# slowkow/harmonypy

Hardware: AMD Instinct MI355X
Metric: cells/sec/Harmony-iteration (higher is better)
Workload: dtype f32; 1 GPU; BASELINE configs[2] (C3): 1000000 cells x 50 PCs, 8 batches, K=100 per GPU; step = 1 Harmony iteration = 10 k-means rounds (block_size 0.05 -> 20 blocks) + 1 ridge correction; cells_per_gpu=1000000, pcs=50, batches=8, clusters=100, update_order=device (keyed bijection, generated inside the timed region), init=k-means++ on a 50k-cell subsample, untimed, parallelism=single GPU, cells_total=1000000

## Files before the change

### harmonypy_amd/_capi.py

```python
from __future__ import annotations

import ctypes as C
import os

import numpy as np

_HERE = os.path.dirname(os.path.abspath(__file__))
LIB_PATH = os.environ.get("HMX_LIB") or os.path.join(_HERE, "libhmx.so")

HMX_TILE = 16
HMX_MAX_CLUSTERS, HMX_MAX_PCS, HMX_MAX_BLOCKS, HMX_MAX_VARS = 320, 320, 250, 32
HMX_Z_ORIG, HMX_Z_COS, HMX_Z_CORR, HMX_R, HMX_Y, HMX_O_GROUP, HMX_T_MASS, HMX_W = range(8)
HMX_ROUND_BLOCK_START, HMX_ROUND_CELLS, HMX_ROUND_TILE_GROUP = 8, 9, 10
HMX_ROUND_CENTROIDS, HMX_ROUND_UPDATE_R, HMX_ROUND_OBJECTIVE = 1, 2, 4
HMX_ROUND_ALL = 7
HMX_DTYPE_F32, HMX_DTYPE_F16, HMX_DTYPE_BF16, HMX_DTYPE_F64 = range(4)

EXPORTS = [
    "hmx_last_error", "hmx_abi_version", "hmx_create", "hmx_destroy", "hmx_upload", "hmx_init_cluster",
    "hmx_cluster_round", "hmx_cluster_round_seeded", "hmx_moe_correct_ridge", "hmx_get", "hmx_set", "hmx_sync", "hmx_device_ptr",
    "hmx_kernel_times", "hmx_enable_timing", "hmx_counters", "hmx_comm_unique_id", "hmx_comm_init", "hmx_set_host_allreduce",
    "hmx_build_id", "hmx_cluster", "hmx_set_timing_stride", "hmx_set_timing_families", "hmx_kmeans_lloyd", "hmx_can_lloyd", "hmx_kmeans_seed", "hmx_compute_lisi", "hmx_get_rows", "hmx_set_ranks", "hmx_peer_export", "hmx_peer_attach", "hmx_peer_selftest", "hmx_peer_enable",
]
DEVICE_IO_EXPORTS = ["hmx_upload_device", "hmx_copy_out_device", "hmx_compute_lisi_device"]
# ... 310 lines not shown
        shape, dt = self._shape(which)
        out = np.empty(shape, dt)
        _check(self._lib.hmx_get(self._h, which, _ptr(out), out.nbytes))
        return out

    def get_rows(self, which, rows):
        rows = _c(rows, np.int32)
        shape, dt = self._shape(which)
        assert dt == np.float32
        out = np.empty((len(rows), shape[1]), np.float32)
        _check(self._lib.hmx_get_rows(self._h, which, _ptr(rows), len(rows), _ptr(out), out.nbytes))
        return out

    def set(self, which, arr):
        shape, dt = self._shape(which)
        arr = _c(arr, dt)
        assert arr.shape == tuple(shape), (arr.shape, shape)
        _check(self._lib.hmx_set(self._h, which, _ptr(arr), arr.nbytes))

    def round_lists(self):
        bs = np.empty(self.nblk + 1, np.int32)
        _check(self._lib.hmx_get(self._h, HMX_ROUND_BLOCK_START, _ptr(bs), bs.nbytes))
        nt = int(bs[-1])
        cells = np.empty(nt * HMX_TILE, np.int32)
        tg = np.empty(nt, np.int32)
        if nt:
            _check(self._lib.hmx_get(self._h, HMX_ROUND_CELLS, _ptr(cells), cells.nbytes))
            _check(self._lib.hmx_get(self._h, HMX_ROUND_TILE_GROUP, _ptr(tg), tg.nbytes))
        return cells, tg, bs

    def sync(self):
        _check(self._lib.hmx_sync(self._h))

    @staticmethod
    def comm_unique_id() -> bytes:
        buf = C.create_string_buffer(HMX_UNIQUE_ID_BYTES)
        _check(load().hmx_comm_unique_id(buf))
        return buf.raw

    def enable_timing(self, on=True, families=None, stride=1):
        _check(self._lib.hmx_set_timing_stride(self._h, int(stride)))
        if on:
            mask = 0xFFFFFFFF if families is None else sum(1 << KERNEL_FAMILIES.index(f) for f in families)
            _check(self._lib.hmx_set_timing_families(self._h, mask))
        _check(self._lib.hmx_enable_timing(self._h, 1 if on else 0))

    def counters(self):
        buf = np.zeros(16, np.int64)
        _check(self._lib.hmx_counters(self._h, _ptr(buf)))
        return {"collectives": int(buf[0]), "sweep_fallbacks": int(buf[1]), "seeded_rounds": int(buf[2]), "sweeps_bf16_pipe": int(buf[3]),
                "sweep_waits": int(buf[4]), "sweep_wait_polls": int(buf[5]), "sweep_wait_polls_max": int(buf[6]), "rtz_bf16_pipe": int(buf[7]),
                "sweeps_group_affine": int(buf[8]), "sweep_group_affine_wgs": int(buf[9]),
                "peer_box": {0: "none", 1: "coarse", 2: "fine"}[int(buf[10])], "rtz_presplit_z": int(buf[11]),
                "sweeps_wide_persistent": int(buf[12]), "rtz_task_tiles_max": int(buf[13])}

    def kernel_times(self):
        buf = np.zeros(2 * len(KERNEL_FAMILIES), np.float64)
        _check(self._lib.hmx_kernel_times(self._h, _ptr(buf), buf.size, None))
        return {n: (float(buf[2 * i]), int(buf[2 * i + 1])) for i, n in enumerate(KERNEL_FAMILIES)}
```

### harmonypy_amd/csrc/hmx_capi.cpp

```cpp
#include <hip/hip_runtime.h>
#include <dlfcn.h>

#include <algorithm>
#include <climits>
#include <cmath>
#include <cstdarg>
#include <cstdio>
#include <cstdlib>
#include <cstring>
#include <functional>
#include <string>
#include <vector>

#include "hmx.h"
#include "hmx_device_io.h"
#include "hmx_knn.h"
#include "hmx_map.h"
#include "hmx_score.h"
#include "hmx_internal.h"
#include "hmx_score_kernels.h"
#ifdef RTZ_PROF
void rtz_prof_dump();
#endif

// ... 55 lines not shown
    hipStream_t s;
    ~SyncOnExit() { (void)hipStreamSynchronize(s); }
};

}

struct hmx_engine {
    hmx_config cfg{};
    int64_t N = 0;
    int d = 0, dp = 0, K = 0, Kp = 0, K16 = 0, mt = 0, ntd = 0, ldy = 0, B = 0, G = 0, V = 0, nblk = 0;
    int max_wgs = 1024;
    hipStream_t stream = nullptr;
    bool uploaded = false, clustered = false, timing = false;
    unsigned timing_mask = ~0u;
    int timing_stride = 1;
    long fam_seen[8] = {0};

    DevBuf<float> Zorig, Zcos, Zcorr, R, Y, Yacc, sigma, theta, Pr_b, lamb, rp, lrp, slab, W;
    DevBuf<int> group_cols, s_cells, s_tile_grp, task_t0, task_t1, task_grp;
    struct Lists { DevBuf<int> cells, tile_grp, blk_start, run_tiles; bool runs_ok = false; };
    Lists lists[2];
    int cur = 0;
    hipStream_t stream2 = nullptr;
    hipEvent_t pre_event = nullptr;
    bool pre_valid = false;
    bool pre_outstanding = false;
    uint64_t pre_seed = 0, pre_counter = 0;
    int64_t pre_cpb = 0;
    DevBuf<int> gstart, chunk_tab, run_count, run_start, global_id;
    DevBuf<int> cell_map, cell_inv;
    bool map_perm = true, inv_valid = false;
    hipEvent_t io_ev[2] = {nullptr, nullptr};
    uint64_t seeded_rounds = 0;
    int64_t Ng = 0;
    DevBuf<double> Ogrp, Tmass, Ohist, scratch;
    DevBuf<double> ref_terms;
    DevBuf<float> km_hn;
    DevBuf<double> km_sums;
    DevBuf<double> Sslots;
    unsigned* sync_words = nullptr;
    unsigned* sync_host = nullptr;
    int n_cus = 0;
    int round_mode = 1;
    unsigned spin_limit = 1u << 24;
    long n_sweep_fallbacks = 0;
    bool lists_beside_rtz = true;
    bool wide_sweep = true;
    bool wide_sweep_launched = false;
    long n_sweeps_wide = 0;
    long n_rtz_bf16 = 0;
    bool allow_round_bf16 = true;
    int rtz3_quad = 4;
    bool allow_rtz_bf16 = true;
    long n_sweeps_bf16 = 0;
    long n_sweeps_ga = 0;
    bool allow_round_ga = true;
    std::vector<int> gsize;
    DevBuf<int> ga_map;
    int ga_nwg = 0;
    int ga_per_wg = 0;
    int64_t ga_key_block = -1;
    int ga_key_cap = -1;
    bool ga_extra = false;
    DevBuf<unsigned long long> wait_stats;
    DevBuf<double> xch;
    double *Sold = nullptr, *Yacc64 = nullptr, *Snew = nullptr, *objacc = nullptr, *Sr = nullptr, *Oxr = nullptr;
    double* obj_host = nullptr;
    double* obj_defer = nullptr;
    hipEvent_t sync_event = nullptr;
    long clean_sweeps = 0;
    long n_sweep_launches = 0;
    long test_fail_sweep = -1;
    unsigned* frozen() const { return reinterpret_cast<unsigned*>(wait_stats.p + 3); }
    void* nccl_comm = nullptr;
    int n_ranks = 1, rank = 0;
    hmx_host_allreduce_fn host_fn = nullptr;
    void* host_ctx = nullptr;
    double* stage_host = nullptr;
    size_t stage_n = 0;
    long n_collectives = 0;
    double* box = nullptr;
    size_t box_doubles = 0;
    bool box_fine = false;
    std::vector<void*> peer_ptrs;
    DevBuf<double*> peer_dev;
    bool peers_attached = false, peers_enabled = false;
    unsigned long long round_epoch = 0;
    unsigned long long selftest_token = 0x5EED0000ull;
    int prefetch_lists = 1;
    int round_wgs_cap = 0;
    int n_s_tiles = 0, ntasks = 0;
    std::vector<int> h_task_grp;
    int rtz3_task_cap = 0;
    int round_req = -1;
    int rtz_kernel = 3;
    bool static_contig = false;
    int ntasks3 = 0;
    int task3_tiles_max = 0;
    DevBuf<int> t3_t0, t3_t1, t3_c0, t3_cend, t3_grp, t3_stride, s_tile_start;
    DevBuf<unsigned char> tile_blk[2], tile_blk_zero;
    DevBuf<unsigned> Yf;
    DevBuf<unsigned> Wf;
    DevBuf<unsigned> Zcf;
    bool zcf_valid = false;
    bool fuse_block_table = true;
    bool allow_zcf = true;
    long n_rtz_zf = 0;
    DevBuf<double> Opriv;
    DevBuf<double> Osave;

    struct Span { hipEvent_t a, b; int fam; };
    std::vector<Span> spans;
    std::vector<hipEvent_t> pool;
    double fam_ms[F_COUNT] = {0};
    long fam_n[F_COUNT] = {0};
};

namespace {

int use_device(hmx_engine* e) {
    HIP_TRY(hipSetDevice(e->cfg.device_id));
    return 0;
}


struct RcclApi {
    void* handle = nullptr;
    int (*GetUniqueId)(void*) = nullptr;
    int (*CommInitRank)(void**, int, hmx_nccl_id, int) = nullptr;
    int (*AllReduce)(const void*, void*, size_t, int, int, void*, hipStream_t) = nullptr;
    int (*CommDestroy)(void*) = nullptr;
    const char* (*GetErrorString)(int) = nullptr;
};
RcclApi g_rccl;

int rccl_load() {
    if (g_rccl.handle) return 0;
    const char* names[] = {getenv("HMX_RCCL_LIB"), "librccl.so.1", "/opt/rocm/lib/librccl.so.1", "librccl.so"};
    void* h = nullptr;
    std::string tried;
    for (const char* n : names) {
        if (!n || !*n) continue;
        h = dlopen(n, RTLD_NOW | RTLD_LOCAL);
        if (h) break;
        tried += std::string(" ") + n + " (" + dlerror() + ")";
    }
    if (!h) return fail(HMX_ERR_COMM, "RCCL not found:%s", tried.c_str());
    RcclApi a;
    a.handle = h;
    a.GetUniqueId = reinterpret_cast<int (*)(void*)>(dlsym(h, "ncclGetUniqueId"));
    a.CommInitRank = reinterpret_cast<int (*)(void**, int, hmx_nccl_id, int)>(dlsym(h, "ncclCommInitRank"));
    a.AllReduce = reinterpret_cast<int (*)(const void*, void*, size_t, int, int, void*, hipStream_t)>(dlsym(h, "ncclAllReduce"));
    a.CommDestroy = reinterpret_cast<int (*)(void*)>(dlsym(h, "ncclCommDestroy"));
// ... 394 lines not shown
        for (int g = 0; g < e->G; ++g) gs[g + 1] = gs[g] + gcount[g];
        if (gs[e->G] != e->N) return fail(HMX_ERR_ARG, "static list must hold every cell exactly once");
        e->gsize = gcount;
        e->ga_nwg = 0; e->ga_key_block = -1;
        if ((rc = e->gstart.reserve(e->G + 1))) return rc;
        HIP_TRY(hipMemcpyAsync(e->gstart.p, gs.data(), gs.size() * sizeof(int), hipMemcpyHostToDevice, e->stream));
        HIP_TRY(hipStreamSynchronize(e->stream));
    }
    std::vector<int> t0, t1, tg;
    const int CH = rtz2_ok(e->mt, e->dp) ? std::max(16, (n_static_tiles + 2 * HMX_RTZ2_WGS_PER_CU * e->n_cus - 1) / (2 * HMX_RTZ2_WGS_PER_CU * e->n_cus))
                   : rtz_wide_ok(e->mt, e->dp) ? std::max(16, (n_static_tiles + 2 * e->n_cus - 1) / (2 * e->n_cus)) : 64;
    for (int i = 0; i < n_static_tiles;) {
        int j = i;
        while (j < n_static_tiles && j - i < CH && static_tile_group[j] == static_tile_group[i]) ++j;
        t0.push_back(i); t1.push_back(j); tg.push_back(static_tile_group[i]);
        i = j;
    }
    for (size_t i = 1; i < tg.size(); ++i)
        if (tg[i] < tg[i - 1]) return fail(HMX_ERR_ARG, "static tiles must be sorted by group");
    e->ntasks = (int)t0.size();
    e->h_task_grp = tg;
    if ((rc = e->task_t0.reserve(t0.size())) || (rc = e->task_t1.reserve(t0.size())) || (rc = e->task_grp.reserve(t0.size()))) return rc;
    HIP_TRY(hipMemcpyAsync(e->task_t0.p, t0.data(), t0.size() * sizeof(int), hipMemcpyHostToDevice, e->stream));
    HIP_TRY(hipMemcpyAsync(e->task_t1.p, t1.data(), t1.size() * sizeof(int), hipMemcpyHostToDevice, e->stream));
    HIP_TRY(hipMemcpyAsync(e->task_grp.p, tg.data(), tg.size() * sizeof(int), hipMemcpyHostToDevice, e->stream));
    {
        bool contig = true;
        std::vector<int> tstart(e->G + 1, 0);
        for (int t = 0; t < n_static_tiles && contig; ++t) {
            const int32_t* c = static_cells + (size_t)t * HMX_TILE;
            int n = 0;
            while (n < HMX_TILE && c[n] >= 0) ++n;
            if (n == 0) { contig = false; break; }
            for (int i = 0; i < HMX_TILE; ++i)
                if (c[i] != (i < n ? c[0] + i : -1)) contig = false;
            const bool last_of_group = t + 1 == n_static_tiles || static_tile_group[t + 1] != static_tile_group[t];
            if (!last_of_group && (n < HMX_TILE || static_cells[(size_t)(t + 1) * HMX_TILE] != c[0] + HMX_TILE)) contig = false;
        }
        for (int t = 0; t < n_static_tiles; ++t) tstart[static_tile_group[t] + 1]++;
        for (int g = 0; g < e->G; ++g) tstart[g + 1] += tstart[g];
        std::vector<int> gs2(e->G + 1, 0);
        {
            std::vector<int> gcount(e->G, 0);
            for (int t = 0; t < n_static_tiles; ++t)
                for (int i = 0; i < HMX_TILE; ++i)
                    if (static_cells[(size_t)t * HMX_TILE + i] >= 0) gcount[static_tile_group[t]]++;
            for (int g = 0; g < e->G; ++g) gs2[g + 1] = gs2[g] + gcount[g];
        }
        for (int g = 0; g < e->G && contig; ++g)
            if (tstart[g + 1] > tstart[g] && static_cells[(size_t)tstart[g] * HMX_TILE] != gs2[g]) contig = false;
        e->static_contig = contig;
        e->ntasks3 = 0;
        e->task3_tiles_max = 0;
        if (contig) {
            std::vector<int> a0, a1, ac0, acend, ag, ast;
            const bool one_per_cu = e->allow_rtz_bf16 && (rtz_wide_ok(e->mt, e->dp) ? rtzw2b_ok(e->mt, e->dp, e->d, e->nblk) : rtz3b_ok(e->mt, e->dp, e->nblk, e->Kp));
            const int target = std::max(1, (one_per_cu ? 1 : 2) * e->n_cus - e->G);
            int cap3 = one_per_cu ? 4096 : 256;
            if (e->rtz3_task_cap) cap3 = e->rtz3_task_cap;
            const int CH3 = std::max(16, std::min(cap3, (n_static_tiles + target - 1) / target));
            e->rtz3_quad = rtz3_quad(e->mt, e->dp, e->nblk, e->Kp, e->allow_rtz_bf16);
            const int quad = rtz_wide_ok(e->mt, e->dp) ? 1 : e->rtz3_quad;
            for (int g = 0; g < e->G; ++g) {
                const int ts = tstart[g], te = tstart[g + 1];
                if (te <= ts) continue;
                const int m = (te - ts + CH3 - 1) / CH3;
                const int mm = std::min(m, (te - ts + quad - 1) / quad);
                const int nq = (te - ts + quad - 1) / quad, first = (nq + mm - 1) / mm;
                e->task3_tiles_max = std::max(e->task3_tiles_max, quad * first - ((nq - 1) % mm == 0 ? quad * nq - (te - ts) : 0));
                for (int j = 0; j < mm; ++j) {
                    a0.push_back(ts + quad * j); a1.push_back(te); ag.push_back(g); ast.push_back(quad * mm);
                    ac0.push_back(gs2[g] + quad * j * HMX_TILE); acend.push_back(gs2[g + 1]);
                }
            }
            e->ntasks3 = (int)a0.size();
            const size_t nt3 = a0.size();
            if ((rc = e->t3_t0.reserve(nt3)) || (rc = e->t3_t1.reserve(nt3)) || (rc = e->t3_c0.reserve(nt3)) || (rc = e->t3_cend.reserve(nt3)) || (rc = e->t3_stride.reserve(nt3)) ||
                (rc = e->t3_grp.reserve(nt3)) || (rc = e->s_tile_start.reserve(e->G + 1)) ||
                (rc = e->tile_blk[0].reserve((size_t)n_static_tiles * HMX_TILE)) || (rc = e->tile_blk[1].reserve((size_t)n_static_tiles * HMX_TILE)) ||
                (rc = e->tile_blk_zero.reserve((size_t)n_static_tiles * HMX_TILE)))
                return rc;
            HIP_TRY(hipMemcpyAsync(e->t3_t0.p, a0.data(), nt3 * sizeof(int), hipMemcpyHostToDevice, e->stream));
            HIP_TRY(hipMemcpyAsync(e->t3_t1.p, a1.data(), nt3 * sizeof(int), hipMemcpyHostToDevice, e->stream));
            HIP_TRY(hipMemcpyAsync(e->t3_c0.p, ac0.data(), nt3 * sizeof(int), hipMemcpyHostToDevice, e->stream));
            HIP_TRY(hipMemcpyAsync(e->t3_stride.p, ast.data(), nt3 * sizeof(int), hipMemcpyHostToDevice, e->stream));
            HIP_TRY(hipMemcpyAsync(e->t3_cend.p, acend.data(), nt3 * sizeof(int), hipMemcpyHostToDevice, e->stream));
            HIP_TRY(hipMemcpyAsync(e->t3_grp.p, ag.data(), nt3 * sizeof(int), hipMemcpyHostToDevice, e->stream));
            HIP_TRY(hipMemcpyAsync(e->s_tile_start.p, tstart.data(), tstart.size() * sizeof(int), hipMemcpyHostToDevice, e->stream));
            HIP_TRY(hipMemsetAsync(e->tile_blk[0].p, 255, (size_t)n_static_tiles * HMX_TILE, e->stream));
            HIP_TRY(hipMemsetAsync(e->tile_blk[1].p, 255, (size_t)n_static_tiles * HMX_TILE, e->stream));
            HIP_TRY(hipMemsetAsync(e->tile_blk_zero.p, 0, (size_t)n_static_tiles * HMX_TILE, e->stream));
            HIP_TRY(hipMemsetAsync(e->R.p + (size_t)e->N * e->Kp, 0, (size_t)16 * e->Kp * sizeof(float), e->stream));
            HIP_TRY(hipMemsetAsync(e->Zorig.p + (size_t)e->N * e->dp, 0, (size_t)16 * e->dp * sizeof(float), e->stream));
            HIP_TRY(hipMemsetAsync(e->Zcos.p + (size_t)e->N * e->dp, 0, (size_t)16 * e->dp * sizeof(float), e->stream));
            HIP_TRY(hipMemsetAsync(e->Zcorr.p + (size_t)e->N * e->dp, 0, (size_t)16 * e->dp * sizeof(float), e->stream));
            HIP_TRY(hipStreamSynchronize(e->stream));
        }
    }
    HIP_TRY(hipStreamSynchronize(e->stream));
    HIP_TRY(hipGetLastError());
    e->uploaded = true;
    return HMX_OK;
}

}

// ... 1205 lines not shown
    if (streaming_rtz(e)) {
        if ((rc = rtz3_pass(e, 1, e->tile_blk_zero.p, 1, false, false, Z))) return rc;
    } else {
    HIP_TRY(hipMemsetAsync(e->Sr, 0, GK * e->ldy * sizeof(double), e->stream));
    HIP_TRY(hipMemsetAsync(e->Oxr, 0, GK * sizeof(double), e->stream));
    {
        Timed t(e, F_RIDGE_STATS);
        RtzArgs r{};
        r.R = e->R.p; r.Z = Z; r.cells = e->s_cells.p; r.tile_grp = e->s_tile_grp.p;
        r.task_tile0 = e->task_t0.p; r.task_tile1 = e->task_t1.p; r.task_grp = e->task_grp.p;
        r.S_out = e->Oxr; r.slab = e->slab.p; r.n_tiles = e->n_s_tiles; r.ntasks = e->ntasks;
        r.K = e->K; r.Kp = e->Kp; r.K16 = e->K16; r.G = e->G; r.mt = e->mt; r.dp = e->dp; r.ntd = e->ntd;
        if (rtz2) {
            launch_rtz2(r, e->ntasks, e->stream);
            launch_rtz2_reduce(e->slab.p, e->ntasks, e->mt, e->dp, e->K16, e->ldy, e->Sr, e->task_grp.p, e->stream);
        } else if (rtzw) {
            launch_rtz_wide(r, e->ntasks, e->stream);
            launch_rtz_wide_reduce(e->slab.p, e->ntasks, e->mt, e->dp, e->K16, e->ldy, e->Sr, e->task_grp.p, e->stream);
        } else {
            launch_rtz(r, (e->ntasks + 3) / 4, e->stream);
            launch_rtz_reduce(e->slab.p, e->ntasks, e->mt, e->ntd, e->K16, e->ldy, e->Sr, e->task_grp.p, e->stream);
        }
    }
    }
    return sum_over_ranks(e, e->Sr, GK * e->ldy + GK);
}

static int ridge_solve_apply(hmx_engine* e, const double* ref_mass, const double* ref_sums) {
    int rc;
    const bool rtz2 = rtz2_ok(e->mt, e->dp);
    const bool rtzw = !rtz2 && rtz_wide_ok(e->mt, e->dp);
    {
        Timed t(e, F_RIDGE_SOLVE);
        RidgeSolveArgs s{};
        s.S = e->Sr; s.Ox = e->Oxr; s.T = e->Tmass.p; s.lamb = e->lamb.p; s.Pr_b = e->Pr_b.p; s.group_cols = e->group_cols.p;
        s.W = e->W.p; s.scratch = e->scratch.p; s.alpha = e->cfg.alpha; s.lambda_est = e->cfg.lambda_estimation;
        s.ref_mass = ref_mass; s.ref_sums = ref_sums;
        s.K = e->K; s.K16 = e->K16; s.G = e->G; s.B = e->B; s.V = e->V; s.d = e->d; s.lds = e->ldy; s.ldw = e->ldy;
        launch_ridge_solve(s, e->stream);
    }
    {
        Timed t(e, F_RIDGE_APPLY);
        ApplyArgs a{};
        a.R = e->R.p; a.Zorig = e->Zorig.p; a.W = e->W.p; a.Zcorr = e->Zcorr.p; a.Zcos = e->Zcos.p;
        a.cells = e->s_cells.p; a.tile_grp = e->s_tile_grp.p; a.n_tiles = e->n_s_tiles;
        a.Kp = e->Kp; a.K16 = e->K16; a.dp = e->dp; a.ldw = e->ldy; a.mtd = e->ntd;
        if (rtz2 || rtzw) { a.task_tile0 = e->task_t0.p; a.task_tile1 = e->task_t1.p; a.task_grp = e->task_grp.p; a.ntasks = e->ntasks; }
        e->zcf_valid = false;
        if (rtzw && e->allow_round_bf16) {
            if ((rc = e->Wf.reserve(w_planes_dwords(e->G, e->K16, e->dp)))) return rc;
            launch_w_planes(e->W.p, e->G, e->K16, e->ldy, e->dp, e->Wf.p, e->stream);
            a.Wf = e->Wf.p;
        }
        if (launch_ridge_apply(a, e->max_wgs, e->stream)) return fail(HMX_ERR_ARG, "unsupported n_pcs");
    }
    HIP_TRY(hipGetLastError());
    return HMX_OK;
}

int hmx_moe_correct_ridge(hmx_engine* e) {
    if (!e) return fail(HMX_ERR_ARG, "null argument");
    if (!e->clustered) return fail(HMX_ERR_STATE, "no soft assignment yet");
    int rc;
    if ((rc = use_device(e))) return rc;
    if ((rc = ridge_stats(e, e->Zorig.p))) return rc;
    return ridge_solve_apply(e, nullptr, nullptr);
}


int hmx_reference_summary(hmx_engine* e, double* cluster_sums_out, double* cluster_mass_out) {
    if (!e || !cluster_sums_out || !cluster_mass_out) return fail(HMX_ERR_ARG, "null argument");
    if (!e->uploaded) return fail(HMX_ERR_STATE, "hmx_upload must come first");
    if (!e->clustered) return fail(HMX_ERR_STATE, "hmx_reference_summary: no soft assignment yet");
    int rc;
    if ((rc = use_device(e))) return rc;
    if ((rc = ridge_stats(e, e->Zcorr.p))) return rc;
    const size_t GK = (size_t)e->G * e->K16, n = GK * e->ldy + GK;
    std::vector<double> h(n);
    HIP_TRY(hipStreamSynchronize(e->stream));
    HIP_TRY(hipGetLastError());
    HIP_TRY(hipMemcpy(h.data(), e->Sr, n * sizeof(double), hipMemcpyDeviceToHost));
    const double* S = h.data();
    const double* O = S + GK * e->ldy;
    for (int k = 0; k < e->K; ++k) {
        double m = 0.0;
        for (int g = 0; g < e->G; ++g) m += O[(size_t)g * e->K16 + k];
        cluster_mass_out[k] = m;
        for (int j = 0; j < e->d; ++j) {
            double v = 0.0;
            for (int g = 0; g < e->G; ++g) v += S[((size_t)g * e->K16 + k) * e->ldy + j];
            cluster_sums_out[(size_t)k * e->d + j] = v;
        }
    }
    return HMX_OK;
}

int hmx_map_query(hmx_engine* e, const double* cluster_sums, const double* cluster_mass) {
    if (!e || !cluster_sums || !cluster_mass) return fail(HMX_ERR_ARG, "null argument");
    if (!e->uploaded) return fail(HMX_ERR_STATE, "hmx_upload must come first");
    const int K = e->K, d = e->d, ldy = e->ldy, K16 = e->K16;
    std::vector<float> y0((size_t)K * d);
    std::vector<double> terms((size_t)K16 * (ldy + 1), 0.0);
    for (int k = 0; k < K; ++k) {
        const double m = cluster_mass[k];
        if (!std::isfinite(m)) return fail(HMX_ERR_ARG, "hmx_map_query: cluster_mass[%d] is not finite", k);
        terms[k] = m;
// ... 126 lines not shown
        const size_t GK = (size_t)e->G * e->K16;
        HIP_TRY(hipMemsetAsync(e->Ogrp.p, 0, GK * sizeof(double), e->stream));
        launch_group_sums(e->R.p, e->Kp, e->K, e->K16, e->s_cells.p, e->s_tile_grp.p, e->n_s_tiles, e->Ogrp.p, e->stream);
        if ((rc = sum_over_ranks(e, e->Ogrp.p, GK))) return rc;
        TableArgs ta = table_args(e);
        ta.O_prev = e->Ogrp.p; ta.T_out = e->Tmass.p;
        launch_block_table(ta, e->K16, e->stream);
        HIP_TRY(hipStreamSynchronize(e->stream));
        HIP_TRY(hipGetLastError());
        e->clustered = true;
    }
    return HMX_OK;
}

int hmx_sync(hmx_engine* e) {
    if (!e) return fail(HMX_ERR_ARG, "null argument");
    int rc;
    if ((rc = use_device(e))) return rc;
    HIP_TRY(hipStreamSynchronize(e->stream));
    HIP_TRY(hipGetLastError());
    return HMX_OK;
}

int hmx_device_ptr(hmx_engine* e, int which, void** d_ptr, size_t* bytes) {
    if (!e || !d_ptr || !bytes) return fail(HMX_ERR_ARG, "null argument");
    size_t need; int rows, cols, ld, elem, rc;
    if ((rc = locate(e, which, d_ptr, &need, &rows, &cols, &ld, &elem))) return rc;
    if (which == HMX_Z_COS) e->allow_zcf = false;
    *bytes = (size_t)rows * ld * elem;
    return HMX_OK;
}

int hmx_counters(hmx_engine* e, int64_t out[HMX_N_COUNTERS]) {
    if (!e || !out) return fail(HMX_ERR_ARG, "null argument");
    int rc;
    if ((rc = use_device(e))) return rc;
    unsigned long long ws[4] = {0, 0, 0, 0};
    HIP_TRY(hipStreamSynchronize(e->stream));
    HIP_TRY(hipMemcpy(ws, e->wait_stats.p, sizeof ws, hipMemcpyDeviceToHost));
    out[0] = e->n_collectives;
    out[1] = e->n_sweep_fallbacks;
    out[2] = (int64_t)e->seeded_rounds;
    out[3] = e->n_sweeps_bf16;
    out[4] = (int64_t)ws[0];
    out[5] = (int64_t)ws[1];
    out[6] = (int64_t)ws[2];
    out[7] = e->n_rtz_bf16;
    out[8] = e->n_sweeps_ga;
    out[9] = e->n_sweeps_ga > 0 ? e->ga_nwg : 0;
    out[10] = e->box ? (e->box_fine ? 2 : 1) : 0;
    out[11] = e->n_rtz_zf;
    out[12] = e->n_sweeps_wide;
    out[13] = e->task3_tiles_max;
    for (int i = 14; i < HMX_N_COUNTERS; ++i) out[i] = 0;
    return HMX_OK;
}

int hmx_enable_timing(hmx_engine* e, int on) {
    if (!e) return fail(HMX_ERR_ARG, "null argument");
    (void)hipSetDevice(e->cfg.device_id);
    (void)hipStreamSynchronize(e->stream);
    drain_spans(e);
    e->timing = on != 0;
    for (int i = 0; i < F_COUNT; ++i) { e->fam_ms[i] = 0; e->fam_n[i] = 0; e->fam_seen[i] = 0; }
    return HMX_OK;
}

int hmx_set_timing_families(hmx_engine* e, unsigned mask) {
    if (!e) return fail(HMX_ERR_ARG, "null argument");
    if (mask == 0) return fail(HMX_ERR_ARG, "empty family mask (hmx_enable_timing(e, 0) turns timing off)");
    e->timing_mask = mask;
    return HMX_OK;
}

int hmx_set_timing_stride(hmx_engine* e, int stride) {
    if (!e || stride < 1) return fail(HMX_ERR_ARG, "stride must be >= 1");
    e->timing_stride = stride;
    return HMX_OK;
}

int hmx_kernel_times(hmx_engine* e, double* ms_out, int n, const char** names_out) {
    if (!e || !ms_out) return fail(HMX_ERR_ARG, "null argument");
    (void)hipSetDevice(e->cfg.device_id);
    (void)hipStreamSynchronize(e->stream);
    drain_spans(e);
    for (int i = 0; i < F_COUNT && 2 * i + 1 < n; ++i) { ms_out[2 * i] = e->fam_ms[i]; ms_out[2 * i + 1] = (double)e->fam_n[i]; }
    if (names_out) *names_out = kFamilyNames;
    return F_COUNT;
}


static int score_engine_checks(hmx_engine* e, int which_Z, const char* who, const float** Z) {
    if (!e->uploaded) return fail(HMX_ERR_STATE, "%s: hmx_upload must come first", who);
    if (!e->clustered) return fail(HMX_ERR_STATE, "%s: no soft assignment yet", who);
    if (sharded(e) || e->n_ranks > 1 || e->Ng != e->N)
        return fail(HMX_ERR_STATE, "%s: this engine holds one shard of a sharded job; mapping confidence needs all cells on one engine", who);
    if (which_Z != HMX_Z_ORIG && which_Z != HMX_Z_CORR) return fail(HMX_ERR_ARG, "%s: which_Z must be HMX_Z_ORIG or HMX_Z_CORR (%d)", who, which_Z);
    *Z = which_Z == HMX_Z_ORIG ? e->Zorig.p : e->Zcorr.p;
    return 0;
}

static int score_chunks(int64_t N, size_t per_chunk, size_t budget, int cap, int64_t* chunk) {
    int64_t c = std::min<int64_t>({(N + 1023) / 1024, (int64_t)(budget / std::max<size_t>(per_chunk, 1)), (int64_t)cap});
    c = std::max<int64_t>(c, 1);
    *chunk = (((N + c - 1) / c) + 7) & ~(int64_t)7;
    return (int)((N + *chunk - 1) / *chunk);
}
// ... 135 lines not shown
```

### harmonypy_amd/csrc/hmx_internal.h

```cpp
#pragma once
#include <hip/hip_runtime.h>
#include <stddef.h>
#include <stdint.h>

#define HMX_RTZ_MTW 7
#define HMX_RTZ_NTW 4
#define HMX_OBJ_SLOTS 64

struct AssignArgs {
    const float* Zcos;
    const float* Y;
    const float* sigma;
    const float* rp;
    const float* lrp;
    float* R;
    const int* cells;
    const int* tile_grp;
    double* S_out;
    double* obj;
    const int* blk_start;
    int blk;
    int tile_begin, tile_end;
    int K, Kp, K16, mt, dp, ldy;
    int G, ldy_lds, tables_in_lds;
// ... 118 lines not shown
void launch_zplanes(const float* Z, int dp, int n_tiles, const int* tile_grp, const int* gstart, const int* s_tile_start, unsigned* Zf, hipStream_t s);
bool rtzw2b_ok(int mt, int dp, int d, int nblk);
int launch_rtzw(const Rtz3Args& a, int mt, int dp, int d, int nblk, hipStream_t s, bool allow_bf16);
void launch_tile_blocks(const int* cells, const int* tile_grp, const int* blk_start, int nblk, int64_t n_pos_upper, const int* gstart,
                        const int* s_tile_start, unsigned char* tile_blk, hipStream_t s);

struct TableArgs {
    const double* O_prev;
    const double* S_add;
    const double* S_sub;
    double* O_out;
    double* T_out;
    float* rp;
    float* lrp;
    double* obj_cross;
    const int* group_cols;
    const float* Pr_b;
    const float* theta;
    const float* sigma;
    int G, B, V, K16;
};

struct RidgeSolveArgs {
    const double* S;
    const double* Ox;
    const double* T;
    const float* lamb;
    const float* Pr_b;
    const int* group_cols;
    float* W;
    double* scratch;
    const double* ref_mass;
    const double* ref_sums;
    float alpha;
    int lambda_est;
    int K, K16, G, B, V, d, lds, ldw;
};

struct ApplyArgs {
    const float* R;
    const float* Zorig;
    const float* W;
    const unsigned* Wf;
    float* Zcorr;
    float* Zcos;
    const int* cells;
    const int* tile_grp;
    int n_tiles;
    int Kp, K16, dp, ldw, mtd;
    const int* task_tile0;
    const int* task_tile1;
    const int* task_grp;
    int ntasks, ldw_lds;
};

struct OrderArgs {
    int64_t N, Ng, cpb;
    const int* global_id;
    int nblk, G, half_bits;
    uint32_t key0, key1;
    const int* gstart;
    int* chunk_tab;
    int* run_count;
    int* run_start;
    int* blk_start;
    int* run_tiles;
    int* cells;
    int* tile_grp;
    unsigned char* tile_blk;
    const int* s_tile_start;
    const unsigned* frozen;
};

size_t round_lds_bytes(int K16, int dp, int G, int B, int V, bool bf3, bool ga, int nblk);
bool round_uses_bf16_pipe(int K16, int dp, int G, int B, int V, bool extra_tiles, bool allow_bf16, bool ga, int nblk);
#define HMX_ROUND_GA_TILES 14
#define HMX_ROUND_GA_MAX_BLOCK_CELLS (1 << 22)
#define HMX_ROUND_LDS_LIMIT (size_t)(159 * 1024)
int round_row_floats(int d);
int launch_round(const RoundArgs& a, int mt, int wgs, hipStream_t s, bool extra_tiles, bool allow_bf16);
size_t peer_box_doubles(int n_ranks, size_t GK);
void launch_peer_selftest(double* const* peer_box, double* my_box, int n_ranks, int rank, size_t GK, unsigned long long token, int iters,
                          unsigned* result, hipStream_t s);
#define LISI_KNN_WAVES 4
#define LISI_MAX_NEIGHBOURS (2048 - 8)
struct LisiKnnArgs {
    const float* X;
    const float* cn;
    int64_t n, npad;
    int dp;
    int cap;
    unsigned long long* lists;
    int* counts;
    unsigned long long* prof;
};
struct LisiFinishArgs {
    const double* X;
    int64_t n;
    int d, nn, n_labels;
    int cap;
    const unsigned long long* lists;
    const int* counts;
    const int* labels;
    double perplexity, tol;
    double* out;
    double* knn_dist;
// ... 103 lines not shown
```

### harmonypy_amd/csrc/hmx_kernels.hip

```cpp
#include <hip/hip_runtime.h>
#include <stdint.h>

#include <algorithm>

#include "hmx_internal.h"
#include "hmx_device.h"
#include <type_traits>

__global__ __launch_bounds__(256) void k_normalize_rows(const float* __restrict__ Z, float* __restrict__ Zc,
                                                        int64_t N, int dp) {
    const int lane16 = threadIdx.x & 15;
    int64_t row = (int64_t)blockIdx.x * 16 + (threadIdx.x >> 4);
    if (row >= N) return;
    const float* z = Z + row * dp;
    float ss = 0.f;
    for (int j = lane16; j < dp; j += 16) ss += z[j] * z[j];
    ss = wave_sum_c16(ss);
    const float nrm = sqrtf(ss);
    float* o = Zc + row * dp;
    for (int j = lane16; j < dp; j += 16) o[j] = z[j] / nrm;
}

template <typename T>
__global__ __launch_bounds__(64) void k_y_normalize(const T* __restrict__ src, float* __restrict__ dst, int K,
// ... 3695 lines not shown
                for (int pn = 0; pn < 3; ++pn) pl[pn] = ld4u(slot + (pn * MTD + mt) * 256);
            };
            auto products = [&](int mt, const u32x4 (&pl)[3]) {
                acc0[mt] = MFMA_BF16(pl[2], bp0[0], acc0[mt]);  acc1[mt] = MFMA_BF16(pl[2], bp1[0], acc1[mt]);
                acc0[mt] = MFMA_BF16(pl[0], bp0[2], acc0[mt]);  acc1[mt] = MFMA_BF16(pl[0], bp1[2], acc1[mt]);
                acc0[mt] = MFMA_BF16(pl[1], bp0[1], acc0[mt]);  acc1[mt] = MFMA_BF16(pl[1], bp1[1], acc1[mt]);
                acc0[mt] = MFMA_BF16(pl[1], bp0[0], acc0[mt]);  acc1[mt] = MFMA_BF16(pl[1], bp1[0], acc1[mt]);
                acc0[mt] = MFMA_BF16(pl[0], bp0[1], acc0[mt]);  acc1[mt] = MFMA_BF16(pl[0], bp1[1], acc1[mt]);
                acc0[mt] = MFMA_BF16(pl[0], bp0[0], acc0[mt]);  acc1[mt] = MFMA_BF16(pl[0], bp1[0], acc1[mt]);
            };
            fetch(0, wp[0]);
#pragma unroll
            for (int mt = 0; mt < MTD; ++mt) {
                if (mt + 1 < MTD) fetch(mt + 1, wp[(mt + 1) & 1]);
                products(mt, wp[mt & 1]);
                __builtin_amdgcn_sched_barrier(0);
                if (mt == 0 && s + 1 < ns) {
                    request(s + 1);
                    load_r(s + 1);
                }
            }
        }
        auto finish = [&](bool has, bool live, int cell, f32x4 (&acc)[MTD]) {
            if (!has) return;
            const size_t row = (size_t)(live ? cell : 0) * a.dp;
            float ss = 0.f;
#pragma unroll
            for (int mt = 0; mt < MTD; ++mt) {
                const int col = 16 * mt + 4 * q;
                const f32x4 zo = (live && col < a.dp) ? ld4(a.Zorig + row + col) : (f32x4){0.f, 0.f, 0.f, 0.f};
                acc[mt] = zo - acc[mt];
#pragma unroll
                for (int r = 0; r < 4; ++r) ss += acc[mt][r] * acc[mt][r];
            }
            ss = wave_sum_q(ss);
            const float nrm = sqrtf(ss);
#pragma unroll
            for (int mt = 0; mt < MTD; ++mt) {
                const int col = 16 * mt + 4 * q;
                if (live && col < a.dp) {
                    st4(a.Zcorr + row + col, acc[mt]);
                    f32x4 zc;
#pragma unroll
                    for (int r = 0; r < 4; ++r) zc[r] = acc[mt][r] / nrm;
                    st4(a.Zcos + row + col, zc);
                }
            }
        };
        finish(has0, live0, cell0, acc0);
        finish(has1, live1, cell1, acc1);
    }
}

__device__ __forceinline__ uint32_t mix32(uint32_t h) {
    h ^= h >> 16; h *= 0x85ebca6bu; h ^= h >> 13; h *= 0xc2b2ae35u; h ^= h >> 16;
    return h;
}
__device__ __forceinline__ uint32_t feistel_position(uint32_t x, uint32_t n, int half_bits, uint32_t k0, uint32_t k1) {
    const uint32_t mask = (1u << half_bits) - 1u;
    do {
        uint32_t l = x >> half_bits, r = x & mask;
#pragma unroll
        for (int i = 5; i >= 0; --i) {
            const uint32_t f = mix32(l * 0x9E3779B1u + k0 + (uint32_t)i * k1) & mask;
            const uint32_t pl = r ^ f;
            r = l;
            l = pl;
        }
        x = (l << half_bits) | r;
    } while (x >= n);
    return x;
}
__device__ __forceinline__ int group_of_cell(const int* __restrict__ gstart, int G, int cell) {
    int lo = 0, hi = G;
    while (hi - lo > 1) {
        const int mid = (lo + hi) >> 1;
        if (gstart[mid] <= cell) lo = mid; else hi = mid;
    }
    return lo;
}

#define ORDER_CHUNK 256

template <int MODE>
__global__ __launch_bounds__(64) void k_order_pass(OrderArgs a) {
    if (a.frozen && *a.frozen) return;
    extern __shared__ int cnt[];
    const int lane = threadIdx.x;
    const int chunk = blockIdx.x, nchunks = gridDim.x;
    const int nkeys = a.nblk * a.G;
    for (int i = lane; i < nkeys; i += 64) cnt[i] = (MODE == 1) ? a.chunk_tab[(size_t)i * nchunks + chunk] : 0;
    __syncthreads();
    int key_bits = 1;
    while ((1 << key_bits) < nkeys) ++key_bits;
    const int64_t base = (int64_t)chunk * ORDER_CHUNK;
    for (int s = 0; s < ORDER_CHUNK / 64; ++s) {
        const int64_t ci = base + s * 64 + lane;
        const bool live = ci < a.N;
        const int cell = (int)ci;
        int key = 0;
        if (live) {
            const uint32_t gid = a.global_id ? (uint32_t)a.global_id[cell] : (uint32_t)cell;
            const int64_t p = feistel_position(gid, (uint32_t)a.Ng, a.half_bits, a.key0, a.key1);
            const int b = (a.cpb > 0) ? (int)min((int64_t)(p / a.cpb), (int64_t)(a.nblk - 1)) : a.nblk - 1;
            const int g = group_of_cell(a.gstart, a.G, cell);
            key = b * a.G + g;
// ... 643 lines not shown
    else hipLaunchKernelGGL(k_ridge_solve_general, dim3(a.K16), dim3(256), 0, s, a);
}

void launch_order(const OrderArgs& a, hipStream_t s) {
    const int nchunks = cdiv(a.N, ORDER_CHUNK);
    const size_t sm = (size_t)a.nblk * a.G * sizeof(int);
    hipLaunchKernelGGL(k_order_pass<0>, dim3(nchunks), dim3(64), sm, s, a);
    hipLaunchKernelGGL(k_order_scan, dim3(a.nblk * a.G), dim3(256), 0, s, a, nchunks);
    hipLaunchKernelGGL(k_order_runs, dim3(a.nblk * a.G), dim3(256), 0, s, a);
    hipLaunchKernelGGL(k_order_pass<1>, dim3(nchunks), dim3(64), sm, s, a);
}

int order_chunks(int64_t N) { return cdiv(N, ORDER_CHUNK); }

void launch_gather_rows(const float* src, int ld, int cols, const int* rows, int n_rows, float* dst, hipStream_t s) {
    if (n_rows <= 0) return;
    hipLaunchKernelGGL(k_gather_rows, dim3(cdiv((int64_t)n_rows * cols, 256)), dim3(256), 0, s, src, ld, cols, rows, n_rows, dst);
}

template <int MTD>
static void launch_apply2_k(const ApplyArgs& a, int kb, size_t sm, hipStream_t s) {
    switch (kb) {
        case 1: hipLaunchKernelGGL((k_ridge_apply2<MTD, 1>), dim3(a.ntasks), dim3(256), sm, s, a); break;
        case 2: hipLaunchKernelGGL((k_ridge_apply2<MTD, 2>), dim3(a.ntasks), dim3(256), sm, s, a); break;
        case 3: hipLaunchKernelGGL((k_ridge_apply2<MTD, 3>), dim3(a.ntasks), dim3(256), sm, s, a); break;
        case 4: hipLaunchKernelGGL((k_ridge_apply2<MTD, 4>), dim3(a.ntasks), dim3(256), sm, s, a); break;
        case 5: hipLaunchKernelGGL((k_ridge_apply2<MTD, 5>), dim3(a.ntasks), dim3(256), sm, s, a); break;
        case 6: hipLaunchKernelGGL((k_ridge_apply2<MTD, 6>), dim3(a.ntasks), dim3(256), sm, s, a); break;
        default: hipLaunchKernelGGL((k_ridge_apply2<MTD, 7>), dim3(a.ntasks), dim3(256), sm, s, a); break;
    }
}

void launch_load_rows(const float* src, int d, const int* source_row, float* dst, int dp, int64_t N, hipStream_t s) {
    if (N <= 0) return;
    hipLaunchKernelGGL(k_load_rows, dim3(cdiv(N * dp, 256)), dim3(256), 0, s, src, d, source_row, dst, dp, N);
}

void launch_kmeans_seed(const SeedArgs& a, int K, hipStream_t s) {
    const int wgs = cdiv(a.n, 256);
    hipLaunchKernelGGL(k_seed_transpose, dim3(cdiv((int64_t)a.n * a.d, 256)), dim3(256), 0, s, a.X, a.n, a.d, a.Xt);
    const size_t sm = (size_t)SEED_TRIALS * a.d * sizeof(float);
    for (int step = 0; step < K; ++step) {
        hipLaunchKernelGGL(k_seed_pick, dim3(1), dim3(256), 0, s, a, step);
        hipLaunchKernelGGL(k_seed_eval, dim3(wgs), dim3(256), sm, s, a, step);
        hipLaunchKernelGGL(k_seed_commit, dim3(wgs), dim3(256), 0, s, a, step);
    }
}

size_t y_planes_dwords(int K16, int dp) { return (size_t)((dp + 31) / 32) * 3 * (K16 / 16) * 256; }
void launch_y_planes(const float* Y, int K16, int ldy, int dp, unsigned* Yf, hipStream_t s) {
    const int ns = (dp + 31) / 32, mt = K16 / 16;
    hipLaunchKernelGGL(k_y_planes, dim3(ns * mt), dim3(64), 0, s, Y, ldy, mt, Yf);
}
size_t w_planes_dwords(int G, int K16, int dp) { return (size_t)G * ((K16 + 31) / 32) * 3 * (dp / 16) * 256; }
void launch_w_planes(const float* W, int G, int K16, int ldw, int dp, unsigned* Wf, hipStream_t s) {
    const int ns = (K16 + 31) / 32, mtd = dp / 16;
    hipLaunchKernelGGL(k_w_planes, dim3(ns * mtd, G), dim3(64), 0, s, W, K16, ldw, mtd, ns, Wf);
}

int launch_ridge_apply(const ApplyArgs& a_in, int max_wgs, hipStream_t s) {
    ApplyArgs a = a_in;
    if (a.n_tiles <= 0) return 0;
    if (a.task_tile0 && a.Wf && rtz_wide_ok((a.K16 + 15) / 16, a.dp)) {
        const int mtd = a.dp / 16;
        const size_t sm = (size_t)2 * 3 * mtd * 1024;
#define HMX_AWB(M)                                                                                                     \
    case M: {                                                                                                         \
        static bool attr_done = false;                                                                                \
        if (!attr_done) {                                                                                             \
            (void)hipFuncSetAttribute(reinterpret_cast<const void*>(k_ridge_apply_wideb<M>), hipFuncAttributeMaxDynamicSharedMemorySize, 80 * 1024); \
            attr_done = true;                                                                                         \
        }                                                                                                             \
        hipLaunchKernelGGL((k_ridge_apply_wideb<M>), dim3(a.ntasks), dim3(64 * APPLYB_WAVES), sm, s, a);               \
    } break;
        if (mtd < 1 || mtd > 13 || sm > (size_t)80 * 1024) return -1;
        switch (mtd) {
            HMX_AWB(1) HMX_AWB(2) HMX_AWB(3) HMX_AWB(4) HMX_AWB(5) HMX_AWB(6) HMX_AWB(7) HMX_AWB(8) HMX_AWB(9) HMX_AWB(10) HMX_AWB(11) HMX_AWB(12)
            HMX_AWB(13)
        }
#undef HMX_AWB
        return 0;
    }
    if (a.task_tile0 && rtz_wide_ok((a.K16 + 15) / 16, a.dp)) {
        const int mtd = a.dp / 16;
        a.ldw_lds = ((16 * mtd + 31) / 32) * 32 + 16;
        const size_t sm = (size_t)2 * 16 * a.ldw_lds * sizeof(float);
#define HMX_AW(M) case M: hipLaunchKernelGGL((k_ridge_apply_wide<M>), dim3(a.ntasks), dim3(64 * WIDE_WAVES), sm, s, a); break;
        switch (mtd) {
            HMX_AW(1) HMX_AW(2) HMX_AW(3) HMX_AW(4) HMX_AW(5) HMX_AW(6) HMX_AW(7) HMX_AW(8) HMX_AW(9) HMX_AW(10) HMX_AW(11) HMX_AW(12)
            default: hipLaunchKernelGGL((k_ridge_apply_wide<13>), dim3(a.ntasks), dim3(64 * WIDE_WAVES), sm, s, a); break;
        }
#undef HMX_AW
        return 0;
    }
    if (a.task_tile0 && rtz2_ok((a.K16 + 15) / 16, a.dp)) {
        const int mtd = a.dp == 32 ? 2 : 4;
        a.ldw_lds = ((16 * mtd + 31) / 32) * 32 + 16;
        const size_t sm = (size_t)a.K16 * a.ldw_lds * sizeof(float);
        if (mtd == 2) launch_apply2_k<2>(a, a.K16 / 16, sm, s);
        else launch_apply2_k<4>(a, a.K16 / 16, sm, s);
        return 0;
    }
    constexpr int NT = 2;
    const int wgs = assign_grid(a.n_tiles, NT, max_wgs);
    if (a.mtd <= 4) hipLaunchKernelGGL((k_ridge_apply<4, NT>), dim3(wgs), dim3(256), 0, s, a);
    else if (a.mtd <= 13) hipLaunchKernelGGL((k_ridge_apply<13, NT>), dim3(wgs), dim3(256), 0, s, a);
    else if (a.mtd <= 20) hipLaunchKernelGGL((k_ridge_apply<20, 1>), dim3(assign_grid(a.n_tiles, 1, max_wgs)), dim3(256), 0, s, a);
    else return -1;
    return 0;
}
```

Measured before the change: 226.8 million cells/sec/Harmony-iteration.

## Add bf16-split MFMA ridge-apply kernel with contiguous per-group task tiling

Adds a new ridge correction apply kernel for the rtz2 shape class (dp 32/64) that splits R into three bf16 planes and multiplies against pre-split W planes held in LDS using bf16 MFMA, replacing the previous fp32 path. It also builds a new contiguous per-group task table sized to about two workgroups per CU, and resizes the W-planes buffer for this case. The aim is to speed up the ridge apply with bf16 matrix throughput while keeping near-fp32 accuracy through the 3-term split. In exchange it adds the W-planes conversion launch and a new host-side task setup.

```diff
diff --git a/harmonypy_amd/_capi.py b/harmonypy_amd/_capi.py
--- a/harmonypy_amd/_capi.py
+++ b/harmonypy_amd/_capi.py
@@ -386,7 +386,8 @@
                 "sweep_waits": int(buf[4]), "sweep_wait_polls": int(buf[5]), "sweep_wait_polls_max": int(buf[6]), "rtz_bf16_pipe": int(buf[7]),
                 "sweeps_group_affine": int(buf[8]), "sweep_group_affine_wgs": int(buf[9]),
                 "peer_box": {0: "none", 1: "coarse", 2: "fine"}[int(buf[10])], "rtz_presplit_z": int(buf[11]),
-                "sweeps_wide_persistent": int(buf[12]), "rtz_task_tiles_max": int(buf[13])}
+                "sweeps_wide_persistent": int(buf[12]), "rtz_task_tiles_max": int(buf[13]),
+                "ridge_apply_bf16_pipe": int(buf[14])}
 
     def kernel_times(self):
         buf = np.zeros(2 * len(KERNEL_FAMILIES), np.float64)
diff --git a/harmonypy_amd/csrc/hmx_capi.cpp b/harmonypy_amd/csrc/hmx_capi.cpp
--- a/harmonypy_amd/csrc/hmx_capi.cpp
+++ b/harmonypy_amd/csrc/hmx_capi.cpp
@@ -131,6 +131,7 @@
     bool allow_round_bf16 = true;
     int rtz3_quad = 4;
     bool allow_rtz_bf16 = true;
+    long n_apply_bf16 = 0;
     long n_sweeps_bf16 = 0;
     long n_sweeps_ga = 0;
     bool allow_round_ga = true;
@@ -178,6 +179,8 @@
     int task3_tiles_max = 0;
     DevBuf<int> t3_t0, t3_t1, t3_c0, t3_cend, t3_grp, t3_stride, s_tile_start;
     DevBuf<unsigned char> tile_blk[2], tile_blk_zero;
+    int ntasks2b = 0;
+    DevBuf<int> t2b_t0, t2b_t1, t2b_grp;
     DevBuf<unsigned> Yf;
     DevBuf<unsigned> Wf;
     DevBuf<unsigned> Zcf;
@@ -678,6 +681,27 @@
         e->static_contig = contig;
         e->ntasks3 = 0;
         e->task3_tiles_max = 0;
+        e->ntasks2b = 0;
+        if (contig && rtz2_ok(e->mt, e->dp)) {
+            std::vector<int> b0, b1, bg;
+            const int target = std::max(1, 2 * e->n_cus - e->G);
+            const int CH2 = std::max(8, (n_static_tiles + target - 1) / target);
+            for (int g = 0; g < e->G; ++g) {
+                const int ts = tstart[g], te = tstart[g + 1];
+                if (te <= ts) continue;
+                const int m = (te - ts + CH2 - 1) / CH2;
+                for (int j = 0; j < m; ++j) {
+                    const int lo = ts + (int)((int64_t)(te - ts) * j / m), hi = ts + (int)((int64_t)(te - ts) * (j + 1) / m);
+                    if (hi > lo) { b0.push_back(lo); b1.push_back(hi); bg.push_back(g); }
+                }
+            }
+            e->ntasks2b = (int)b0.size();
+            if ((rc = e->t2b_t0.reserve(b0.size())) || (rc = e->t2b_t1.reserve(b0.size())) || (rc = e->t2b_grp.reserve(b0.size()))) return rc;
+            HIP_TRY(hipMemcpyAsync(e->t2b_t0.p, b0.data(), b0.size() * sizeof(int), hipMemcpyHostToDevice, e->stream));
+            HIP_TRY(hipMemcpyAsync(e->t2b_t1.p, b1.data(), b0.size() * sizeof(int), hipMemcpyHostToDevice, e->stream));
+            HIP_TRY(hipMemcpyAsync(e->t2b_grp.p, bg.data(), b0.size() * sizeof(int), hipMemcpyHostToDevice, e->stream));
+            HIP_TRY(hipStreamSynchronize(e->stream));
+        }
         if (contig) {
             std::vector<int> a0, a1, ac0, acend, ag, ast;
             const bool one_per_cu = e->allow_rtz_bf16 && (rtz_wide_ok(e->mt, e->dp) ? rtzw2b_ok(e->mt, e->dp, e->d, e->nblk) : rtz3b_ok(e->mt, e->dp, e->nblk, e->Kp));
@@ -1989,6 +2013,14 @@
             launch_w_planes(e->W.p, e->G, e->K16, e->ldy, e->dp, e->Wf.p, e->stream);
             a.Wf = e->Wf.p;
         }
+        if (rtz2 && e->allow_round_bf16 && e->static_contig && e->ntasks2b > 0) {
+            if ((rc = e->Wf.reserve(w_planes_dwords(e->G, e->K16, e->dp)))) return rc;
+            launch_w_planes(e->W.p, e->G, e->K16, e->ldy, e->dp, e->Wf.p, e->stream);
+            a.Wf = e->Wf.p;
+            a.task_tile0 = e->t2b_t0.p; a.task_tile1 = e->t2b_t1.p; a.task_grp = e->t2b_grp.p; a.ntasks = e->ntasks2b;
+            a.gstart = e->gstart.p; a.s_tile_start = e->s_tile_start.p;
+            e->n_apply_bf16++;
+        }
         if (launch_ridge_apply(a, e->max_wgs, e->stream)) return fail(HMX_ERR_ARG, "unsupported n_pcs");
     }
     HIP_TRY(hipGetLastError());
@@ -2221,7 +2253,8 @@
     out[11] = e->n_rtz_zf;
     out[12] = e->n_sweeps_wide;
     out[13] = e->task3_tiles_max;
-    for (int i = 14; i < HMX_N_COUNTERS; ++i) out[i] = 0;
+    out[14] = e->n_apply_bf16;
+    for (int i = 15; i < HMX_N_COUNTERS; ++i) out[i] = 0;
     return HMX_OK;
 }
 
diff --git a/harmonypy_amd/csrc/hmx_internal.h b/harmonypy_amd/csrc/hmx_internal.h
--- a/harmonypy_amd/csrc/hmx_internal.h
+++ b/harmonypy_amd/csrc/hmx_internal.h
@@ -194,6 +194,8 @@
     const int* task_tile1;
     const int* task_grp;
     int ntasks, ldw_lds;
+    const int* gstart;
+    const int* s_tile_start;
 };
 
 struct OrderArgs {
diff --git a/harmonypy_amd/csrc/hmx_kernels.hip b/harmonypy_amd/csrc/hmx_kernels.hip
--- a/harmonypy_amd/csrc/hmx_kernels.hip
+++ b/harmonypy_amd/csrc/hmx_kernels.hip
@@ -3771,6 +3771,122 @@
     }
 }
 
+template <int MTD, int KSN>
+__global__ __launch_bounds__(256, 2) void k_ridge_apply2b(ApplyArgs a) {
+    extern __shared__ __attribute__((aligned(16))) unsigned char smem[];
+    unsigned* Wl = reinterpret_cast<unsigned*>(smem);
+    const int tid = threadIdx.x, lane = tid & 63, wv = tid >> 6;
+    const int c16 = lane & 15, q = lane >> 4;
+    const int task = blockIdx.x;
+    if (task >= a.ntasks) return;
+    const int t0 = a.task_tile0[task], t1 = a.task_tile1[task], g = a.task_grp[task];
+    const int c_first = a.gstart[g] + 16 * (t0 - a.s_tile_start[g]), c_end = a.gstart[g + 1];
+    {
+        const u32x4* src = reinterpret_cast<const u32x4*>(a.Wf + (size_t)g * (KSN * 3 * MTD * 256));
+        for (int i = tid; i < KSN * 3 * MTD * 64; i += 256) reinterpret_cast<u32x4*>(Wl)[i] = src[i];
+    }
+    __syncthreads();
+    const unsigned* frag = Wl + 4 * lane;
+    const f32x4 zero = {0.f, 0.f, 0.f, 0.f};
+    f32x4 rv[KSN][4];
+    const int lcol = 32 * (KSN - 1) + 8 * q;
+    const bool lk0 = lcol < a.Kp, lk1 = lcol + 4 < a.Kp;
+    auto load_r = [&](int t, int s) {
+        const int ta = min(t, t1 - 1), tb = min(t + 1, t1 - 1);
+        const float* r0 = a.R + (size_t)(c_first + 16 * (ta - t0) + c16) * a.Kp;
+        const float* r1 = a.R + (size_t)(c_first + 16 * (tb - t0) + c16) * a.Kp;
+        const int ca = (s < KSN - 1 || lk0) ? 32 * s + 8 * q : 0, cb = (s < KSN - 1 || lk1) ? 32 * s + 8 * q + 4 : 0;
+        __builtin_amdgcn_sched_barrier(0);
+        rv[s][0] = ld4(r0 + ca);
+        rv[s][1] = ld4(r0 + cb);
+        rv[s][2] = ld4(r1 + ca);
+        rv[s][3] = ld4(r1 + cb);
+        __builtin_amdgcn_sched_barrier(0);
+    };
+    auto split4 = [&](const f32x4& lo, const f32x4& hi, u32x4 (&pl)[3]) {
+        unsigned h, m, l;
+        bf16_split3((f32x2){lo[0], lo[1]}, h, m, l); pl[0][0] = h; pl[1][0] = m; pl[2][0] = l;
+        bf16_split3((f32x2){lo[2], lo[3]}, h, m, l); pl[0][1] = h; pl[1][1] = m; pl[2][1] = l;
+        bf16_split3((f32x2){hi[0], hi[1]}, h, m, l); pl[0][2] = h; pl[1][2] = m; pl[2][2] = l;
+        bf16_split3((f32x2){hi[2], hi[3]}, h, m, l); pl[0][3] = h; pl[1][3] = m; pl[2][3] = l;
+    };
+    const int t_first = t0 + 2 * wv;
+    if (t_first >= t1) return;
+#pragma unroll
+    for (int s = 0; s < KSN; ++s) load_r(t_first, s);
+    for (int t = t_first; t < t1; t += 8) {
+        const int cell[2] = {c_first + 16 * (t - t0) + c16, c_first + 16 * (t - t0) + 16 + c16};
+        const bool live[2] = {cell[0] < c_end, t + 1 < t1 && cell[1] < c_end};
+        f32x4 zo[2][MTD];
+#pragma unroll
+        for (int n = 0; n < 2; ++n) {
+            const float* zr = a.Zorig + (size_t)(c_first + 16 * (min(t + n, t1 - 1) - t0) + c16) * a.dp;
+#pragma unroll
+            for (int mt = 0; mt < MTD; ++mt) zo[n][mt] = ld4(zr + min(16 * mt + 4 * q, a.dp - 4));
+        }
+        f32x4 acc0[MTD], acc1[MTD];
+#pragma unroll
+        for (int mt = 0; mt < MTD; ++mt) acc0[mt] = acc1[mt] = zero;
+#pragma unroll
+        for (int s = 0; s < KSN; ++s) {
+            u32x4 bp0[3], bp1[3];
+            if (s == KSN - 1) {
+                rv[s][0] = lk0 ? rv[s][0] : zero; rv[s][2] = lk0 ? rv[s][2] : zero;
+                rv[s][1] = lk1 ? rv[s][1] : zero; rv[s][3] = lk1 ? rv[s][3] : zero;
+            }
+            split4(rv[s][0], rv[s][1], bp0);
+            split4(rv[s][2], rv[s][3], bp1);
+            load_r(t + 8, s);
+            const unsigned* slot = frag + s * (3 * MTD * 256);
+            u32x4 wp[2][3];
+            auto fetch = [&](int mt, u32x4 (&pl)[3]) {
+#pragma unroll
+                for (int pn = 0; pn < 3; ++pn) pl[pn] = ld4u(slot + (pn * MTD + mt) * 256);
+            };
+            auto products = [&](int mt, const u32x4 (&pl)[3]) {
+                acc0[mt] = MFMA_BF16(pl[2], bp0[0], acc0[mt]);  acc1[mt] = MFMA_BF16(pl[2], bp1[0], acc1[mt]);
+                acc0[mt] = MFMA_BF16(pl[0], bp0[2], acc0[mt]);  acc1[mt] = MFMA_BF16(pl[0], bp1[2], acc1[mt]);
+                acc0[mt] = MFMA_BF16(pl[1], bp0[1], acc0[mt]);  acc1[mt] = MFMA_BF16(pl[1], bp1[1], acc1[mt]);
+                acc0[mt] = MFMA_BF16(pl[1], bp0[0], acc0[mt]);  acc1[mt] = MFMA_BF16(pl[1], bp1[0], acc1[mt]);
+                acc0[mt] = MFMA_BF16(pl[0], bp0[1], acc0[mt]);  acc1[mt] = MFMA_BF16(pl[0], bp1[1], acc1[mt]);
+                acc0[mt] = MFMA_BF16(pl[0], bp0[0], acc0[mt]);  acc1[mt] = MFMA_BF16(pl[0], bp1[0], acc1[mt]);
+            };
+            fetch(0, wp[0]);
+#pragma unroll
+            for (int mt = 0; mt < MTD; ++mt) {
+                if (mt + 1 < MTD) fetch(mt + 1, wp[(mt + 1) & 1]);
+                products(mt, wp[mt & 1]);
+                __builtin_amdgcn_sched_barrier(0);
+            }
+        }
+        auto finish = [&](bool lv, int c, const f32x4 (&z)[MTD], f32x4 (&acc)[MTD]) {
+            const size_t row = (size_t)c * a.dp;
+            float ss = 0.f;
+#pragma unroll
+            for (int mt = 0; mt < MTD; ++mt) {
+                acc[mt] = (16 * mt + 4 * q < a.dp ? z[mt] : zero) - acc[mt];
+#pragma unroll
+                for (int r = 0; r < 4; ++r) ss += acc[mt][r] * acc[mt][r];
+            }
+            ss = wave_sum_q(ss);
+            const float nrm = sqrtf(ss);
+#pragma unroll
+            for (int mt = 0; mt < MTD; ++mt) {
+                const int col = 16 * mt + 4 * q;
+                if (lv && col < a.dp) {
+                    st4(a.Zcorr + row + col, acc[mt]);
+                    f32x4 zc;
+#pragma unroll
+                    for (int r = 0; r < 4; ++r) zc[r] = acc[mt][r] / nrm;
+                    st4(a.Zcos + row + col, zc);
+                }
+            }
+        };
+        finish(live[0], cell[0], zo[0], acc0);
+        finish(live[1], cell[1], zo[1], acc1);
+    }
+}
+
 __device__ __forceinline__ uint32_t mix32(uint32_t h) {
     h ^= h >> 16; h *= 0x85ebca6bu; h ^= h >> 13; h *= 0xc2b2ae35u; h ^= h >> 16;
     return h;
@@ -4520,10 +4636,22 @@
     const int ns = (dp + 31) / 32, mt = K16 / 16;
     hipLaunchKernelGGL(k_y_planes, dim3(ns * mt), dim3(64), 0, s, Y, ldy, mt, Yf);
 }
-size_t w_planes_dwords(int G, int K16, int dp) { return (size_t)G * ((K16 + 31) / 32) * 3 * (dp / 16) * 256; }
+static int w_planes_tiles(int K16, int dp) { return rtz2_ok((K16 + 15) / 16, dp) ? (dp == 32 ? 2 : 4) : dp / 16; }
+size_t w_planes_dwords(int G, int K16, int dp) { return (size_t)G * ((K16 + 31) / 32) * 3 * w_planes_tiles(K16, dp) * 256; }
 void launch_w_planes(const float* W, int G, int K16, int ldw, int dp, unsigned* Wf, hipStream_t s) {
-    const int ns = (K16 + 31) / 32, mtd = dp / 16;
+    const int ns = (K16 + 31) / 32, mtd = w_planes_tiles(K16, dp);
     hipLaunchKernelGGL(k_w_planes, dim3(ns * mtd, G), dim3(64), 0, s, W, K16, ldw, mtd, ns, Wf);
+}
+
+template <int MTD>
+static void launch_apply2b_k(const ApplyArgs& a, int ns, hipStream_t s) {
+    const size_t sm = (size_t)ns * 3 * MTD * 1024;
+    switch (ns) {
+        case 1: hipLaunchKernelGGL((k_ridge_apply2b<MTD, 1>), dim3(a.ntasks), dim3(256), sm, s, a); break;
+        case 2: hipLaunchKernelGGL((k_ridge_apply2b<MTD, 2>), dim3(a.ntasks), dim3(256), sm, s, a); break;
+        case 3: hipLaunchKernelGGL((k_ridge_apply2b<MTD, 3>), dim3(a.ntasks), dim3(256), sm, s, a); break;
+        default: hipLaunchKernelGGL((k_ridge_apply2b<MTD, 4>), dim3(a.ntasks), dim3(256), sm, s, a); break;
+    }
 }
 
 int launch_ridge_apply(const ApplyArgs& a_in, int max_wgs, hipStream_t s) {
@@ -4561,6 +4689,12 @@
 #undef HMX_AW
         return 0;
     }
+    if (a.task_tile0 && a.Wf && rtz2_ok((a.K16 + 15) / 16, a.dp)) {
+        if (!a.gstart || !a.s_tile_start) return -1;
+        if (a.dp == 32) launch_apply2b_k<2>(a, (a.K16 + 31) / 32, s);
+        else launch_apply2b_k<4>(a, (a.K16 + 31) / 32, s);
+        return 0;
+    }
     if (a.task_tile0 && rtz2_ok((a.K16 + 15) / 16, a.dp)) {
         const int mtd = a.dp == 32 ? 2 : 4;
         a.ldw_lds = ((16 * mtd + 31) / 32) * 32 + 16;
```

After: 223.7 million cells/sec/Harmony-iteration. 1.4% lower.
